# isabella232/kyverno

Measured on AMD Instinct MI355X. Metric: resource×rule validate evals/sec (node), higher is better.
Workload: dtype u8; 1 GPU; C2: synthetic Pods x 100 validate.pattern rules (image globs, ?*, quantities, |-lists); rules=100, pairs_per_gpu=100000000, output=full, parallelism=resource-shard x1, engine=specialized

## Files before the change

kyverno_amd/csrc/kvdevfn.h:

```cpp
#pragma once

#define KV_SENT 0xFFFFFFFFu


#ifdef KV_JIT_PRELUDE
#define KV_FN __device__ __forceinline__
#define KV_GLOB_FN __device__ __forceinline__
#else
#define KV_FN __device__
#define KV_GLOB_FN __device__ __noinline__
#endif

__device__ __forceinline__ uint32_t uni(uint32_t v) { return __builtin_amdgcn_readfirstlane(v); }

#ifndef KV_SCONST
#define KV_SCONST __attribute__((address_space(4)))
#endif
template <class T>
__device__ __forceinline__ T sld(const T* p) {
  static_assert(sizeof(T) % 4 == 0, "sld: whole words");
  const KV_SCONST uint32_t* q = (const KV_SCONST uint32_t*)p;
  uint32_t w[sizeof(T) / 4];
#pragma unroll
  for (uint32_t i = 0; i < sizeof(T) / 4; i++) w[i] = q[i];
// ... 601 lines not shown
  uint32_t kind, flags, pn, key, res, i0, i1, i2, i3;
};

__device__ __forceinline__ uint2 err8_pack(uint32_t kind, uint32_t flags, uint32_t pn, uint32_t key, uint32_t i0,
                                           uint32_t i1, uint32_t i2, uint32_t i3, uint32_t r) {
  const uint32_t fits = (i0 < 1024u) & (i1 < 256u) & (i2 < 256u) & (i3 == 0u) & (key == ABSENT) & (pn < (1u << 25));
  uint2 w;
  w.x = kind | (flags << 4) | ((fits ^ 1u) << 6) | (pn << 7);
  w.y = (i0 & 1023u) | ((i1 & 255u) << 10) | ((i2 & 255u) << 18) | ((r & 63u) << 26);
  return w;
}

__device__ __forceinline__ void store_err(const DevOut& O, uint32_t ri, uint32_t n_res, uint32_t r, uint32_t kind,
                                          uint32_t flags, uint32_t pn, uint32_t key, uint32_t res, uint32_t i0,
                                          uint32_t i1, uint32_t i2, uint32_t i3) {
#if defined(KV_JIT_PRELUDE) && !defined(KVEMU)
  if (KV_OFULL(O) & 4) return;
#else
  if (KV_OFULL(O) & 4) {
    uint4* x = (uint4*)(O.err + (size_t)ri * n_res) + 2u * r;
    x[0] = make_uint4(kind | (flags << 16), pn, key, res);
    x[1] = make_uint4(i0, i1, i2, i3);
    return;
  }
#endif
  ((uint2*)(O.err8 + (size_t)ri * n_res))[r] = err8_pack(kind, flags, pn, key, i0, i1, i2, i3, r);
}

__device__ __forceinline__ uint32_t kv_count_bytes(uint32_t w, uint32_t b4) {
  const uint32_t t = w ^ b4;
  return (uint32_t)__popc(~(((t & 0x7F7F7F7Fu) + 0x7F7F7F7Fu) | t | 0x7F7F7F7Fu));
}

__device__ __forceinline__ uint32_t kv_ptab_col(const DevPS& P, uint32_t type, uint32_t a) {
  if (type - 1u < 4u) return a;
  return P.n_vals - KV_PTAB_PSEUDO + (type == NT_NULL ? 0u : type == NT_MAP ? 1u : 2u);
}

__device__ __forceinline__ uint32_t kv_leaf_word(const DevPS& P, const Node* __restrict__ N, const Node& n, uint32_t w) {
  const uint32_t t = node_type(n.kt);
#ifdef KV_DIAG_XPTAB
  if (t != NT_ARR) return (n.a * 0x9E3779B9u) ^ (w * 0x85EBCA6Bu);
#endif
  if (t != NT_ARR) return kv_gld(P.ptab, (size_t)w * P.n_vals + kv_ptab_col(P, t, n.a));
  uint32_t x = 0xFFFFFFFFu;
  for (uint32_t k = 0; k < n.b; k++) {
    const Node e = N[ni(n.a + k)];
    x &= kv_gld(P.ptab, (size_t)w * P.n_vals + kv_ptab_col(P, node_type(e.kt), e.a));
  }
  return x;
}

__device__ __forceinline__ uint32_t kv_leaf_word_n(const DevPS& P, const Node* __restrict__ N, const Node& n, uint32_t w) {
  const uint32_t t = node_type(n.kt);
  if (t != NT_ARR) return kv_leaf_word(P, N, n, w);
  const uint32_t ai = ni(n.a);
  const uint32_t first = kv_gld(&N[ai].a, 0), count = kv_gld(&N[ai].b, 0);
  uint32_t x = 0xFFFFFFFFu;
  for (uint32_t k = 0; k < count; k++) {
    const Node e = N[ni(first + k)];
    x &= kv_gld(P.ptab, (size_t)w * P.n_vals + kv_ptab_col(P, node_type(e.kt), e.a));
  }
  return x;
}

__device__ __forceinline__ void kv_rec_put(const DevOut& O, uint32_t ri, uint32_t n_res, uint32_t r, uint32_t slot,
                                           const EState& e, uint32_t z) {
#ifdef KV_DIAG_NORECST
  asm volatile("" ::"v"(slot));
  return;
#endif
  ((uint2*)(O.err8 + (size_t)ri * n_res))[(r & ~63u) + (slot & 63u)] =
      err8_pack(e.kind + z, e.flags, e.pn + z, e.key + z, e.i0, e.i1, e.i2, e.i3, r);
}

__device__ __forceinline__ void kv_final(const DevOut& O, uint32_t ri, uint32_t n_res, uint32_t r, bool valid,
                                         uint32_t st, const EState& e, uint8_t* s_row, uint32_t row) {
#ifdef KV_DIAG_NOREC
  if (false) {
#else
  if (valid && (KV_OFULL(O) & 2) && (st == ST_FAIL || st == ST_ERROR || st == ST_SKIP)) {
#endif
    uint32_t z = 0u;
#ifndef KVEMU
    asm volatile("" : "+v"(r), "+v"(z));
    asm volatile("" : "+s"(ri));
#endif
#if defined(KV_JIT_PRELUDE) && !defined(KVEMU)
    if (!(KV_OFULL(O) & 4)) {
      uint8_t* s_c = s_row - KV_ROW0 - row * KV_RSTRIDE + __builtin_amdgcn_readfirstlane(threadIdx.x >> 6) * KV_KROWS;
      const uint32_t sh = 8u * (row & 3u);
      kv_rec_put(O, ri, n_res, r, atomicAdd((uint32_t*)(s_c + (row & ~3u)), 1u << sh) >> sh, e, z);
    }
#else
    store_err(O, ri, n_res, r, e.kind + z, e.flags, e.pn + z, e.key + z, e.res + z, e.i0, e.i1, e.i2, e.i3);
#endif
// ... 257 lines not shown
```

kyverno_amd/csrc/kvjit.hpp:

```cpp
#pragma once
#include <cstdint>
#include <map>
#include <string>
#include <vector>

#include "kvinternal.hpp"
#include "kvdevtypes.h"

namespace kvh {

struct JitChunk {
  std::vector<uint32_t> rules;
  std::string name;
};

struct JitKernelPlan {
  uint32_t first, count;
  int waves;
  std::vector<uint32_t> blocks;
};

struct JitImage {
  std::vector<JitKernelPlan> plan;
  std::string source;
  std::string common;
  std::vector<std::string> kernel_name, kernel_src;
  std::vector<std::vector<char>> codes;
  std::vector<JitChunk> chunks;
  std::vector<uint32_t> memo_preds;
  uint32_t memo_words = 0;
  uint32_t ptab_row = 1;
  uint32_t mtup_words = 0;
  std::vector<uint32_t> fac_word, fac_bit, fac_flist, fac_rule;
  uint32_t fac_slots = 0;
  std::vector<uint8_t> rec_compact;
  std::vector<uint32_t> gs_desc, gs_mem;
  uint32_t gs_members = 0;
  std::vector<kv::ColDesc> cols;
  std::vector<uint32_t> fam_arr, fam_ncols;
  std::vector<uint32_t> fam_nw, fam_nb, fam_nn;
  std::map<std::string, uint32_t> col_use;
  bool probe = false;
  double gen_ms = 0, compile_ms = 0;
  struct Variant {
    uint32_t full = 0;
    std::vector<std::vector<char>> codes;
  };
  std::vector<Variant> variants;
};

uint32_t jit_chunk_rules();
constexpr uint32_t kJitStamps = 16;
// ... 19 lines not shown
```

kyverno_amd/csrc/kvjitbuild.cpp:

```cpp
#include <hip/hiprtc.h>

#include <dlfcn.h>
#include <sched.h>
#include <spawn.h>
#include <sys/stat.h>
#include <sys/wait.h>

#include <cerrno>
#include <unistd.h>

#include <algorithm>
#include <atomic>
#include <chrono>
#include <cstdio>
#include <cstdlib>
#include <cstring>
#include <set>
#include <sstream>
#include <stdexcept>
#include <thread>

#include "kvjit.hpp"

extern char** environ;
// ... 236 lines not shown
bool reg_verdict(const JitImage& img, size_t ci, int waves, RegVerdict* out) {
  uint32_t priv = 0, vgprs = 0;
  if (ci >= img.codes.size() || !co_kernel_info(img.codes[ci], img.kernel_name[ci], &priv, &vgprs)) return false;
  *out = reg_verdict_of(priv, vgprs, waves, img.kernel_src[ci].find("kv_dleaf_impl") != std::string::npos);
  return true;
}

std::string variant_common(const JitImage& img, uint32_t full) {
  return "#define KVJ_FULL " + std::to_string(full) + "u\n" + img.common;
}

}

RegVerdict reg_verdict_of(uint32_t priv, uint32_t vgprs, int waves, bool calls) {
  RegVerdict v{priv, vgprs, calls, false, false};
  v.fits = waves == 0 || vgprs <= 512u / (uint32_t)waves;
  v.scratch_ok = priv == 0 || (calls && waves == 0);
  return v;
}

bool jit_plan_spills(JitImage* img, const std::vector<RegVerdict>& verdicts) {
  std::vector<JitKernelPlan> next;
  bool changed = false;
  for (size_t k = 0; k < img->plan.size(); k++) {
    const JitKernelPlan& kp = img->plan[k];
    const RegVerdict& v = verdicts.at(k);
    if (v.ships()) {
      next.push_back(kp);
      continue;
    }
    changed = true;
    JitKernelPlan np = kp;
    const size_t big = (size_t)(std::max_element(np.blocks.begin(), np.blocks.end()) - np.blocks.begin());
    if (v.calls && v.fits) {
      np.waves = 0;
    } else if (kp.waves > 6 && np.blocks.size() > 1) {
      np.waves = kp.waves - 1;
    } else if (!np.blocks.empty() && np.blocks[big] > 1) {
      const uint32_t c = np.blocks[big], h = c / 2;
      np.blocks[big] = h;
      np.blocks.insert(np.blocks.begin() + big + 1, c - h);
    } else if (kp.waves > 1) {
      np.waves = kp.waves - 1;
    } else if (kp.waves == 1) {
      np.waves = 0;
    } else if (kp.count > 1) {
      const uint32_t h = kp.count / 2;
      next.push_back({kp.first, h, 0, std::vector<uint32_t>(h, 1u)});
      next.push_back({kp.first + h, kp.count - h, 0, std::vector<uint32_t>(kp.count - h, 1u)});
      continue;
    } else {
      throw std::runtime_error("kvjit: kernel " + img->chunks[k].name + " needs " + std::to_string(v.priv) +
                               " B of scratch per lane even without a launch bound");
    }
    next.push_back(np);
  }
  if (changed) img->plan = next;
  return changed;
}

namespace {

bool jit_plan_spills(JitImage* img) {
  std::vector<RegVerdict> verdicts(img->plan.size());
  for (size_t k = 0; k < img->plan.size(); k++)
    if (!reg_verdict(*img, program_of(*img, img->chunks[k].name), img->plan[k].waves, &verdicts[k]))
      throw std::runtime_error("kvjit: no kernel descriptor for " + img->chunks[k].name);
// ... 66 lines not shown
        else nb.push_back(c);
      }
      img->plan[k].blocks = nb;
    }
  }
}

std::string jit_plan_key(const JitImage& img) {
  uint64_t h = common_hash(img.common);
  for (size_t i = 0; i < img.kernel_src.size(); i++) h = fnv1a64(img.kernel_src[i], fnv1a64(img.kernel_name[i], h));
  char key[40];
  snprintf(key, sizeof key, "%016llx", (unsigned long long)h);
  return key;
}

}

uint64_t code_bytes(const JitImage& img) {
  uint64_t n = 0;
  for (auto& c : img.codes) n += c.size();
  return n;
}

bool jit_load_plan(const std::string& key, JitImage* img) {
  const std::string dir = cache_dir();
  std::vector<char> text;
  if (dir.empty() || !read_file(dir + "/plan-" + key + ".txt", &text)) return false;
  std::vector<JitKernelPlan> plan;
  std::istringstream in(std::string(text.begin(), text.end()));
  for (std::string line; std::getline(in, line);) {
    if (line.rfind("kernel ", 0) != 0) continue;
    std::istringstream ls(line.substr(7));
    JitKernelPlan kp{0, 0, 0, {}};
    ls >> kp.first >> kp.count >> kp.waves;
    uint32_t sum = 0;
    for (uint32_t b; ls >> b; sum += b) kp.blocks.push_back(b);
    if (sum != kp.count || kp.blocks.empty()) return false;
    plan.push_back(kp);
  }
  if (plan.empty()) return false;
  img->plan = plan;
  return true;
}

void jit_save_plan(const std::string& key, const JitImage& img) {
  const std::string dir = cache_dir();
  if (dir.empty()) return;
  std::string t;
  for (const JitKernelPlan& kp : img.plan) {
    t += "kernel " + std::to_string(kp.first) + " " + std::to_string(kp.count) + " " + std::to_string(kp.waves);
    for (uint32_t b : kp.blocks) t += " " + std::to_string(b);
    t += "\n";
  }
  const uint64_t hc = common_hash(img.common);
  for (size_t i = 0; i < img.kernel_src.size(); i++) t += "co " + cache_file(img, i, hc) + "\n";
  for (const JitImage::Variant& v : img.variants) {
    const uint64_t hv = common_hash(variant_common(img, v.full));
    for (size_t i = 0; i < img.kernel_src.size(); i++)
      if (i < v.codes.size() && !v.codes[i].empty()) t += "co " + cache_file(img, i, hv) + "\n";
  }
  write_file_atomic(dir, dir + "/plan-" + key + ".txt", t);
}

void jit_build(const PolicySet& ps, JitImage* img) {
  const uint32_t chunk = jit_chunk_rules();
  const char* dump = getenv("KVGPU_JIT_DUMP");
  jit_generate(ps, chunk, img);
  if (dump) write_file(dump, img->source);
  if (!getenv("KVGPU_JIT_SKIP_COMPILE")) {
    const std::string pkey = jit_plan_key(*img);
    if (!jit_load_plan(pkey, img)) jit_refine_blocks(ps, chunk, img);
    jit_generate(ps, chunk, img);
    bool settled = false;
    for (int round = 0; round < 64 && !settled; round++) {
      jit_compile(img);
      settled = !jit_plan_spills(img);
      if (!settled) jit_generate(ps, chunk, img);
    }
    if (!settled)
      throw std::runtime_error("kvjit: the register plan did not settle (kernels still spill after 64 re-plans)");
    jit_compile_variants(img);
    jit_save_plan(pkey, *img);
    if (dump) write_file(dump, img->source);
  }
  if (const char* co = getenv("KVGPU_JIT_DUMP_CO")) {
    for (size_t i = 0; i < img->codes.size(); i++) write_file(std::string(co) + "." + img->kernel_name[i] + ".co", img->codes[i]);
    for (const JitImage::Variant& v : img->variants)
      for (size_t i = 0; i < v.codes.size(); i++)
        if (!v.codes[i].empty())
          write_file(std::string(co) + "." + img->kernel_name[i] + ".m" + std::to_string(v.full) + ".co", v.codes[i]);
  }
}

}
```

kyverno_amd/csrc/kvjitgen.cpp:

```cpp
#include <algorithm>
#include <chrono>
#include <cstdio>
#include <cstdlib>
#include <cstring>
#include <map>
#include <set>
#include <sstream>
#include <stdexcept>
#include <unordered_map>

#include "kvjit.hpp"
#include "kvdevtypes.h"

namespace kvh {

using namespace kv;

namespace {

const char* kPrelude =
#include "kvjit_prelude.inc"
    ;

std::string hex32(uint32_t v) {
// ... 46 lines not shown
  struct Form {
    std::string text;
    std::vector<uint32_t> preds, pns;
    std::vector<uint32_t> leafpcs;
  };

  const PolicySet& ps;
  const GenOpts opt;

  std::vector<uint32_t> mpreds;
  std::map<uint32_t, uint32_t> pslot;
  std::map<uint32_t, uint32_t> pmask;
  std::vector<Fam> fams;
  std::map<std::string, uint32_t> fam_of;
  std::map<std::string, uint32_t> use_seed;
  std::vector<uint32_t> gs_desc, gs_mem;
  uint32_t gs_members = 0;
  std::vector<uint32_t> mt_bits;
  std::vector<uint8_t> rec_slot;
  uint32_t gtab_n = 0;
  std::map<uint32_t, Form> forms;
  std::map<uint32_t, uint32_t> bslot;
  std::map<uint32_t, std::set<uint32_t>> glob_bytes;
  std::vector<std::pair<std::string, std::string>> helpers;
  std::set<uint32_t> globs_done, atoms_done, preds_done, blks_done;
  std::set<std::pair<char, uint32_t>> qglobs_done, qatoms_done, qpreds_done;
  bool dleaf_done = false;
  std::vector<std::pair<std::string, std::string>> kernels;

  struct Kern {
    uint32_t mt_kbase = 0;
    uint32_t gs0 = 0, gsn = 0;
    std::string decls;
  };

  explicit Gen(const PolicySet& p) : ps(p), rec_slot(p.rules.size(), 0) {
    fams.emplace_back();
    col_of(0, "R");
  }

  struct Helper : std::ostringstream {
    Gen& g;
    const std::string name;
    Helper(Gen& gg, std::string n) : g(gg), name(std::move(n)) {}
    ~Helper() { g.helpers.push_back({name, str()}); }
  };
  static std::string num(const char* prefix, uint32_t i) { return prefix + std::to_string(i); }

  enum ColUse : uint32_t { CU_WIDE = 1u, CU_B = 2u, CU_LEAF = 4u };
  void col_mark(int fam, uint32_t j, uint32_t use) {
    if (fam >= 0 && j != kNoCol) fams.at((size_t)fam).use.at(j) |= use;
  }
  static std::string col_macro(const char* what, uint32_t f, uint32_t j) {
    return std::string("KVC_") + what + "_" + std::to_string(f) + "_" + std::to_string(j);
  }
  static constexpr uint32_t kNoCol = 0xFFFFFFFFu;
  static bool expr_steps(const std::string& ex, std::vector<uint32_t>* out) {
    out->clear();
    size_t at = ex.find('/');
    while (at != std::string::npos) {
      const size_t nx = ex.find('/', at + 1);
      const std::string tok = ex.substr(at + 1, nx == std::string::npos ? std::string::npos : nx - at - 1);
      if (tok.size() < 2 || (tok[0] != 's' && tok[0] != 'k')) return false;
      const unsigned long v = strtoul(tok.c_str() + 1, nullptr, 10);
      if (v >= KV_COL_SCAN) return false;
      out->push_back((uint32_t)v | (tok[0] == 'k' ? KV_COL_SCAN : 0u));
// ... 3 lines not shown
  }
  uint32_t col_of(uint32_t f, const std::string& rel) {
    Fam& F = fams.at(f);
    auto it = F.idx.find(rel);
    if (it != F.idx.end()) return it->second;
    std::vector<uint32_t> st;
    if (!expr_steps(rel, &st)) return kNoCol;
    const uint32_t j = (uint32_t)F.steps.size();
    F.idx.emplace(rel, j);
    F.steps.push_back(st);
    F.use.push_back(0u);
    return j;
  }
  uint32_t family(const std::string& arr) {
    auto it = fam_of.find(arr);
    if (it != fam_of.end()) return it->second;
    if (col_of(0, arr) == kNoCol) return kNoCol;
    const uint32_t f = (uint32_t)fams.size();
    fams.emplace_back();
    fams.back().arr = arr;
    col_of(f, "");
    fam_of.emplace(arr, f);
    return f;
  }
  void col_plan(JitImage* out, std::string* defs) const {
    out->cols.clear();
    out->fam_arr.clear();
    out->fam_ncols.clear();
    out->fam_nw.clear();
    out->fam_nb.clear();
    out->fam_nn.clear();
    out->col_use.clear();
    std::ostringstream d;
    for (uint32_t f = 0; f < fams.size(); f++) {
      const Fam& F = fams[f];
      out->fam_arr.push_back(f ? fams[0].idx.at(F.arr) : 0u);
      out->fam_ncols.push_back((uint32_t)F.steps.size());
      std::vector<uint32_t> use(F.steps.size(), 0u);
      for (const auto& kv : F.idx) {
        const std::string key = F.arr + "|" + kv.first;
        uint32_t u = F.use[kv.second];
        auto it = use_seed.find(key);
        if (it != use_seed.end()) u |= it->second;
        if (f == 0 && fam_of.count(kv.first)) u |= CU_WIDE | CU_B;
        use[kv.second] = u;
        out->col_use[key] = u;
      }
      uint32_t nw = 0, nb = 0, nn = 0;
      const size_t c0 = out->cols.size();
      for (uint32_t j = 0; j < F.steps.size(); j++) {
        ColDesc c{};
        c.fam = f;
        c.j = j;
        c.nsteps = (uint32_t)F.steps[j].size();
        for (uint32_t s = 0; s < c.nsteps; s++) c.steps[s] = F.steps[j][s];
        if (opt.narrow && !(use[j] & CU_WIDE)) {
          c.fmt = KV_COLF_NARROW;
          c.pos = nn++;
        } else {
          c.pos = nw++;
          c.fmt = KV_COLF_WIDE;
          if (use[j] & (CU_B | CU_LEAF)) {
            c.fmt = KV_COLF_WIDEB;
            c.bpos = nb++;
          }
        }
        out->cols.push_back(c);
      }
      out->fam_nw.push_back(nw);
      out->fam_nb.push_back(nb);
      out->fam_nn.push_back(nn);
      d << "#define KVC_W" << f << " " << (3u * nw + nb + nn) * KV_LANES << "u\n";
      for (uint32_t j = 0; j < F.steps.size(); j++) {
        const ColDesc& c = out->cols[c0 + j];
        d << "#define " << col_macro("LD", f, j) << "(b) ";
        if (c.fmt == KV_COLF_NARROW) {
          d << "kv_ldn(PC, (b) + " << u32((3u * nw + nb + c.pos) * KV_LANES) << " + ln_)\n"
            << "#define " << col_macro("IX", f, j) << "(n) (node_type((n).kt) == NT_MAP ? KV_NARROW_IDX : 0u)\n"
            << "#define " << col_macro("LW", f, j) << "(n, w) kv_leaf_word_n(P, N, n, w)\n";
        } else {
          if (c.fmt == KV_COLF_WIDEB)
            d << "kv_ldwb(PC, (b) + " << u32(c.pos * 3u * KV_LANES) << " + 3u * ln_, (b) + "
              << u32((3u * nw + c.bpos) * KV_LANES) << " + ln_)\n";
          else
            d << "kv_ldw(PC, (b) + " << u32(c.pos * 3u * KV_LANES) << " + 3u * ln_)\n";
          d << "#define " << col_macro("IX", f, j) << "(n) (node_type((n).kt) == NT_MAP ? (n).c : 0u)\n"
            << "#define " << col_macro("LW", f, j) << "(n, w) kv_leaf_word(P, N, n, w)\n";
        }
      }
    }
    for (uint32_t f = 1; f < fams.size(); f++) out->cols.at(out->fam_arr[f]).arr_fam = f;
    *defs = d.str();
  }

  template <class Fn>
  void each_atom(uint32_t pi, Fn fn) const {
    const Pred& pr = ps.preds[pi];
    if (pr.kind != PK_STRING) return;
    for (uint32_t a = pr.first; a < pr.first + pr.count; a++)
      for (uint32_t c = ps.alts[a].first; c < ps.alts[a].first + ps.alts[a].count; c++) {
        fn(ps.conjs[c].a0);
        if (ps.conjs[c].kind != CJ_ATOM) fn(ps.conjs[c].a1);
      }
  }

  std::string seg_expr(const GSeg& sg, const std::string& k, bool aligned0) {
    const uint32_t nw = (sg.len + 3) / 4;
    std::ostringstream e;
    e << "([&]() -> bool { ";
    if (aligned0) {
      e << "uint32_t x = 0u; ";
      for (uint32_t i = 0; i < nw; i++) {
        const GWord& g = ps.gwords[sg.wfirst + i];
        if (g.mask == 0) continue;
        e << "x |= (base[" << i << "] ^ " << hex32(g.w) << ") & " << hex32(g.mask) << "; ";
      }
      e << "return x == 0u; })()";
      return e.str();
    }
    e << "const uint32_t k_ = " << k << ", a_ = k_ >> 2, sh_ = k_ & 3u; uint32_t lo_ = base[a_], hi_, x = 0u; ";
// ... 542 lines not shown
    for (uint32_t f = rr.m_first; f < rr.m_first + rr.m_count; f++) blk_fn(f);
    for (uint32_t f = rr.x_first; f < rr.x_first + rr.x_count; f++) blk_fn(f);
    auto call = [&](uint32_t f) { return "g_blk_" + std::to_string(f) + "(P, B, R, rkind, rflags)"; };
    auto combine = [&](uint32_t mode, uint32_t first, uint32_t count) {
      std::ostringstream e;
      if (mode == 0 || count == 0) {
        e << call(first);
      } else {
        e << "(";
        for (uint32_t f = first; f < first + count; f++) e << (f > first ? (mode == 1 ? " || " : " && ") : "") << call(f);
        e << ")";
      }
      return e.str();
    };
    Helper o(*this, num("g_match_", ri));
    o << "__device__ __forceinline__ bool " << o.name
      << "(const DevPS& P, const DevBatch& B, const Res* __restrict__ R, uint32_t rkind, uint32_t rflags) {\n"
      << "  if (!" << combine(rr.m_mode, rr.m_first, rr.m_count) << ") return false;\n"
      << "  return !" << combine(rr.x_mode, rr.x_first, rr.x_count) << ";\n}\n";
  }

  static uint32_t prog_end(const PolicySet& ps, uint32_t pc) {
    while ((ps.prog[pc].op & 0xFF) != OP_DONE) pc++;
    return pc;
  }

  static constexpr uint32_t FIN = 0x7F000000u, ACT = 0x80000000u;

  struct HVar {
    std::string idx, node;
    int fam = -1;
    uint32_t j = kNoCol;
  };
  struct HoistTable {
    std::string prefix;
    std::map<std::string, HVar> vars;
    std::vector<std::string> code;
    std::set<std::string> words;
    size_t flushed = 0;
    uint32_t n = 0;
    int fam = -1;
    std::string troot, cell0;
    std::string flush() {
      std::string s;
      for (; flushed < code.size(); flushed++) s += code[flushed];
      return s;
    }
  };

  struct RGen {
    uint32_t ri = 0, b = 0, e = 0, maxd = 1;
    std::vector<std::pair<uint32_t, uint32_t>> loops;
    std::vector<std::string> expr;
    std::vector<HVar> hv;
    std::vector<std::vector<std::pair<int, uint32_t>>> csrc;
    std::set<uint32_t> resume;
    std::set<uint32_t> carry_ok, carry_err;
    std::vector<char> lean, post_alt;
    std::vector<uint32_t> post_flags, skip_to;
    uint32_t q = 0;
    bool uses_anchor = false, uses_keyglob = false;
    bool grp = false;
    uint32_t gn = 1, grow = 0, gsri = 0, gspn = 0;
    std::vector<uint32_t> gri, gdpn;
    std::map<uint32_t, uint32_t> gslot;
    std::string gtab;
    bool gsite = false;
    uint32_t gl = 0, gpre = 0;
    uint32_t max_level = 0;
    std::string s;
  };

  HVar hoist(HoistTable& T, const std::string& pexpr, const HVar& p, uint32_t a, uint32_t aux) {
    const bool scan = (aux & AUX_SCAN) != 0;
    const std::string ex = pexpr + (scan ? "/k" : "/s") + std::to_string(a);
    auto it = T.vars.find(ex);
    if (it != T.vars.end()) return it->second;
    HVar h{T.prefix + "h" + std::to_string(T.n), T.prefix + "hn" + std::to_string(T.n)};
    T.n++;
    std::ostringstream c;
    const uint32_t j = T.fam >= 0 ? col_of((uint32_t)T.fam, T.fam == 0 ? ex : ex.substr(T.troot.size())) : kNoCol;
    if (j != kNoCol) {
      h.fam = T.fam;
      h.j = j;
      c << "  const Node " << h.node << " = " << col_macro("LD", (uint32_t)T.fam, j) << "(" << T.cell0 << ");\n"
        << "  const uint32_t " << h.idx << " = " << h.node << ".kt == 0u ? ABSENT : "
        << col_macro("IX", (uint32_t)T.fam, j) << "(" << h.node << ");\n";
      T.code.push_back(c.str());
      T.vars.emplace(ex, h);
      return h;
    }
    col_mark(p.fam, p.j, CU_WIDE | CU_B);
    c << "  uint32_t " << h.idx << " = ABSENT; Node " << h.node << "{0u, 0u, 0u, 0u};\n";
    if (scan) {
      c << "  if (node_type(" << p.node << ".kt) == NT_MAP) for (uint32_t q_ = 0u; q_ < " << p.node << ".b; q_++) { "
        << "const uint32_t c_ = ni(" << p.node << ".a + q_); const Node t_ = N[c_]; if (node_key(t_.kt) == " << u32(a)
        << ") { " << h.idx << " = c_; " << h.node << " = t_; break; } }\n";
    } else {
      c << "  { const bool ok_ = node_type(" << p.node << ".kt) == NT_MAP && " << u32(a) << " < " << p.node << ".b; "
        << "const uint32_t c_ = ok_ ? ni(" << p.node << ".a + " << u32(a) << ") : 0u; const Node t_ = N[c_]; "
        << "const bool hit_ = ok_ && node_type(t_.kt) != NT_ABSENT; const uint32_t m_ = hit_ ? 0x07060504u : 0x0c0c0c0cu; "
        << h.idx << " = hit_ ? c_ : ABSENT; " << h.node << " = Node{__builtin_amdgcn_perm(t_.kt, 0u, m_), "
        << "__builtin_amdgcn_perm(t_.a, 0u, m_), __builtin_amdgcn_perm(t_.b, 0u, m_), __builtin_amdgcn_perm(t_.c, 0u, m_)}; }\n";
    }
    T.code.push_back(c.str());
    T.vars.emplace(ex, h);
    return h;
  }

  struct Region {
    int kind = 0;
    uint32_t rb = 0, re = 0;
    uint32_t jre = 0;
    std::string se;
    std::set<uint32_t>*jumps = nullptr, *err_jumps = nullptr;
    std::string li0;
    HoistTable* T = nullptr;
    std::string troot;
  };

  struct GInfo {
    std::vector<uint32_t> members, pns0, leafpcs;
    std::vector<uint32_t> dpn;
    std::vector<std::vector<uint32_t>> preds;
  };

  struct Block {
    Kern& kern;
    const uint32_t hbase;
    std::vector<uint32_t> rules;
    std::vector<GInfo> ginfo;
    std::map<uint32_t, size_t> gof;
    std::vector<RGen> gs;
    HoistTable global;
    size_t K = 0;
    Block(Kern& k, uint32_t hb) : kern(k), hbase(hb) {
      global.prefix = "g";
      global.fam = 0;
// ... 152 lines not shown
        case OP_KEYGLOB:
          if (G) throw std::runtime_error("kvjit: KEYGLOB in a rule group");
          set_unknown(d + 1);
          IDX(d);
          w << "  { uint32_t nd_; if (!keyglob_op(P, B, N, " << cd << ", " << u32(in.op) << ", " << u32(in.a) << ", "
            << u32(in.c) << ", &nd_, &kn" << s << ")) " << jump(in.b) << " " << cn << " = nd_; }\n";
          break;
        case OP_SCOPE_END:
          if (G) break;
          if (in.c == 0) w << "  if (" << kindof << ") " << ek << " |= " << u32(aux << 4) << ";\n";
          else w << "  if (" << kindof << ") { " << ek << " |= " << u32(aux << 4) << "; " << jump(in.c, true) << " }\n";
          break;
        case OP_POS_END:
          if (G) throw std::runtime_error("kvjit: POS_END in a rule group");
          w << "  if (" << kindof << ") { if (" << ek << " & " << u32(EF_COND << 4) << ") " << ek << " = 0u; else "
            << jump(in.c, true) << " }\n";
          break;
        case OP_NEG:
          w << "  if (" << lookup(d, in.a, aux, false) << " != ABSENT) " << raise(E_NEG, in.b, in.c) << "\n";
          break;
        case OP_STAR:
          w << "  if (" << absent_or(d + 1, "== NT_NULL") << ") " << raise(E_STAR, in.b, in.c) << "\n";
          break;
        case OP_LEAF: {
          const uint32_t slot = G ? g.gslot.at(pc) : slot_for(in.a);
          const uint32_t word = slot / 32;
          HoistTable* T = known(d) ? table_for(d) : nullptr;
          std::string wx;
          if (T) {
            const HVar& hvd = g.hv[d];
            const std::string hn = hvd.node;
            wx = hn + "_w" + std::to_string(word);
            col_mark(hvd.fam, hvd.j, CU_LEAF);
            if (T->words.insert(wx).second)
              T->code.push_back("  const uint32_t " + wx + " = " +
                                (hvd.fam >= 0 ? col_macro("LW", (uint32_t)hvd.fam, hvd.j) + "(" + hn + ", "
                                              : "kv_leaf_word(P, N, " + hn + ", ") +
                                u32(word) + ");\n");
          } else {
            IDX(d);
            wx = "kv_leaf_word(P, N, (" + cd + " != ABSENT ? N[" + cd + "] : Node{0u, 0u, 0u, 0u}), " + u32(word) + ")";
          }
          if (G) {
            const uint32_t mask = g.gn >= 32 ? 0xFFFFFFFFu : (1u << g.gn) - 1u;
            w << "  { const uint32_t f_ = " << al << " & ~((" << wx << " >> " << u32(slot % 32) << ") & " << hex32(mask)
              << ");\n    if (f_) { " << gfin("f_", E_VALUE, in.b, in.c) << " " << al << " &= ~f_; if (!" << al << ") "
              << gdone() << " } }\n";
          } else {
            w << "  if (!(((" << wx << " >> " << u32(slot % 32) << ") & 1u) != 0u)) " << raise(E_VALUE, in.b, in.c) << "\n";
          }
          break;
        }
        case OP_VLEAF:
          if (G) throw std::runtime_error("kvjit: VLEAF in a rule group");
          if (known(d)) w << "  { const Node vn_ = " << NODE(d, CU_WIDE | CU_B) << ";\n";
          else {
            IDX(d);
            w << "  { Node vn_{0u, 0u, 0u, 0u}; if (" << cd << " != ABSENT) vn_ = N[" << cd << "];\n";
          }
          dleaf_fn();
          w << "    if (!g_dleaf_0(B, N, B.dleaf[(size_t)" << u32(in.a) << " * n_res + r], vn_)) "
            << raise(E_VALUE, in.b, in.c) << " }\n";
          break;
        case OP_RAISE:
          w << "  " << raise(in.b, in.a, in.c) << "\n";
          break;
        case OP_EXISTCHK:
          w << "  if (" << absent_or(d, "!= NT_ARR") << ") " << raise(E_EXIST_RESTYPE, in.a, in.c) << "\n";
          break;
        case OP_LENCHK:
          w << "  if (" << NODE(d, CU_WIDE | CU_B) << ".b < " << u32(in.a) << ") " << raise(E_LEN, in.b, in.c) << "\n";
// ... 557 lines not shown
    }
    Loop L;
    L.k = k;
    L.tag = tag;
    L.troot = "E" + tag;
    L.T.prefix = "l" + tag + "_";
    L.fam = key[0] == 'R' && fams[0].idx.count(key) ? family(key) : kNoCol;
    if (L.fam != kNoCol) {
      L.T.fam = (int)L.fam;
      L.T.troot = L.troot;
      L.T.cell0 = "ec" + tag;
    }
    std::ostringstream bodies;
    for (RGen* gp : grp) loop_body(B, *gp, L, bodies);
    std::vector<uint32_t> gmask(B.mask_words(), 0);
    for (const RGen* gp : grp)
      if (gp->lean[k]) gmask[gp->q / 32] |= 1u << (gp->q % 32);
    body << "  { // fused loop " << tag << " over " << key << " (" << grp.size() << " rules)\n"
         << "    uint32_t fn" << tag << " = 0u, ff" << tag << " = 0u, fe" << tag << " = 0u;\n    if (((0u";
    for (const RGen* gp : grp)
      if (!gp->lean[k]) body << " | rs" << gp->s;
    body << ") & ACT_)";
    for (uint32_t w = 0; w < gmask.size(); w++)
      if (gmask[w]) body << " | (am" << k << "_" << w << " & " << u32(gmask[w]) << ")";
    body << ") { const Node an_ = " << arr_node << "; ff" << tag << " = an_.a; fn" << tag << " = an_.b; fe" << tag
         << " = an_.c; }\n";
    body << "    for (uint32_t fli" << tag << " = 0u; fli" << tag << " < fn" << tag << "; fli" << tag << "++) {\n"
         << "      const uint32_t el" << tag << " = ni(ff" << tag << " + fli" << tag << ");\n";
    if (L.fam != kNoCol)
      body << "      const uint32_t ec" << tag << " = fe" << tag << " + fli" << tag << " * KVC_W" << L.fam
           << ";\n      const Node eln" << tag << " = " << col_macro("LD", L.fam, 0) << "(ec" << tag << ");\n";
    else
      body << "      const Node eln" << tag << " = N[el" << tag << "];\n";
    body << L.T.flush() << bodies.str() << "    }\n";
    for (const RGen* gp : grp)
      if (!gp->lean[k]) body << "    rs" << gp->s << " &= ~ACT_;\n";
    body << "  }\n";
  }

  void emit_fused_loops(Block& B, size_t k, std::ostream& body) {
    std::map<std::string, std::vector<RGen*>> groups;
    std::vector<std::string> order;
    for (RGen& g : B.gs) {
      if (k >= g.loops.size()) continue;
      const uint32_t d = (ps.prog[g.loops[k].first].op >> 8) & 0xFF;
      const std::string key = g.expr[d].empty() ? "U" + std::to_string(g.ri) : g.expr[d];
      if (!groups.count(key)) order.push_back(key);
      groups[key].push_back(&g);
    }
    uint32_t li = 0;
    for (const std::string& key : order) emit_fused_loop(B, k, key, groups[key], std::to_string(k) + "_" + std::to_string(li++), body);
  }

  void emit_rule_state(const Block& B, std::ostream& k) const {
    for (uint32_t ri : B.rules)
      if (!B.gof.count(ri)) k << "  uint32_t rs_" << ri << " = FIN_ | ST_NOMATCH;\n";
    for (const RGen& g : B.gs) {
      const std::string& s = g.s;
      if (g.grp) k << "  uint32_t rs" << s << " = FIN_ | ST_STORED_, al" << s << " = 0u;\n";
      k << "  uint32_t ek" << s << " = 0u";
      for (uint32_t lv = 0; lv <= g.max_level && lv < 4; lv++) k << ", ei" << lv << s << " = 0u";
      if (g.uses_keyglob) k << ", kn" << s << " = ABSENT, ekn" << s << " = ABSENT";
      k << ";\n";
      if (g.uses_anchor) k << "  uint64_t areg" << s << " = 0ull, apres" << s << " = 0ull;\n";
      k << "  uint32_t c0" << s << " = root";
      for (uint32_t d = 1; d < g.maxd; d++) k << ", c" << d << s << " = ABSENT";
      k << ";\n";
      k << "  uint32_t";
      for (uint32_t l = 0; l <= g.max_level && l < 4; l++)
        k << (l ? "," : "") << " li" << l << s << " = 0u, lf" << l << s << " = 0u, ll" << l << s << " = 0u";
      k << ";\n";
    }
  }

  static void check_resumes(const Block& B) {
    for (const RGen& g : B.gs)
      for (uint32_t t : g.resume) {
        bool ok = false;
        for (size_t k = 0; k <= g.loops.size() && !ok; k++) ok = t >= segment(g, k).first && t < segment(g, k).second;
        if (!ok) throw std::runtime_error("kvjit: resume target " + std::to_string(t) + " of rule " +
                                         std::to_string(g.ri) + " is not in a segment");
      }
  }

  std::string fused_block(Kern& kern, const std::vector<uint32_t>& rules_in, uint32_t hbase, std::vector<uint32_t>* order) {
    Block B(kern, hbase);
    form_groups(rules_in, &B);
    *order = B.rules;
    prepare_rules(&B);
    std::ostringstream body;
    for (size_t k = 0; k <= B.K; k++) {
      std::ostringstream seg;
      for (RGen& g : B.gs)
        if (k <= g.loops.size()) emit_segment(B, g, k, seg);
      if (k < B.K) {
        body << "  uint32_t";
        for (uint32_t w = 0; w < B.mask_words(); w++)
          body << (w ? "," : "") << " am" << k << "_" << w << " = 0u, sk" << k << "_" << w << " = 0u";
        body << ";\n";
      }
      body << B.global.flush() << seg.str();
      if (k < B.K) emit_fused_loops(B, k, body);
    }
    check_resumes(B);
    std::ostringstream k;
    emit_rule_state(B, k);
    for (uint32_t q = 0; q < B.rules.size(); q++)
      if (no_program(ps.rules[B.rules[q]])) k << match_code(B, q) << store(B, q);
    k << body.str();
    return k.str();
  }

  static uint32_t kernel_lds(uint32_t nr) { return KV_ROW0 + nr * KV_RSTRIDE; }
  static int lds_waves(uint32_t nr) {
    const uint32_t g = 1280u, b = (kernel_lds(nr) + g - 1u) / g * g;
    return (int)std::max<uint32_t>(1u, (160u * 1024u) / std::max(b, g) * KV_RWAVES / 4u);
  }
  std::vector<uint32_t> group_kernel(const std::string& name, const std::vector<std::vector<uint32_t>>& chs, int waves) {
    std::vector<std::string> blocks;
    std::vector<std::pair<uint32_t, uint32_t>> rows;
    std::vector<uint32_t> rules;
    uint32_t nr_all = 0;
    for (const auto& c : chs) nr_all += (uint32_t)c.size();
    if (nr_all > KV_KROWS) throw std::runtime_error("kvjit: at most KV_KROWS rules per kernel (KVGPU_JIT_CHUNK)");
    Kern kern;
    kern.mt_kbase = (uint32_t)(mt_bits.size() / 32u);
    kern.gs0 = (uint32_t)(gs_desc.size() / 4u);
    for (const auto& c : chs) {
      std::vector<uint32_t> ord;
      rows.push_back({(uint32_t)rules.size(), (uint32_t)c.size()});
      blocks.push_back(fused_block(kern, c, (uint32_t)rules.size(), &ord));
      rules.insert(rules.end(), ord.begin(), ord.end());
    }
    mt_bits.insert(mt_bits.end(), rules.begin(), rules.end());
    while (mt_bits.size() % 32u) mt_bits.push_back(0xFFFFFFFFu);
    const uint32_t nr = (uint32_t)rules.size();
    if (kern.gsn > 64u) throw std::runtime_error("kvjit: more than 64 site-record groups in one kernel");
    std::ostringstream o;
    o << kern.decls;
    if (opt.stamps) o << "__device__ unsigned long long* kvj_stamps;\n";
    o << "__device__ const uint32_t " << name << "_rules[" << nr << "] = {";
    for (uint32_t q = 0; q < nr; q++) o << (q ? ", " : "") << u32(rules[q]);
    o << "};\n";
    const std::string lb = waves > 0 ? "KV_RWG, " + std::to_string(waves) : "KV_RWG";
    o << "extern \"C\" __global__ __launch_bounds__(" << lb << ") void " << name
      << "(const DevPS* __restrict__ Pp, const DevBatch* __restrict__ Bp, const Node* __restrict__ N, "
         "const Val* __restrict__ V, const uint8_t* __restrict__ S, DevOut O, uint32_t r0) {\n"
      << "  constexpr uint32_t FIN_ = " << u32(FIN) << ", ACT_ = " << u32(ACT) << ", ST_STORED_ = 0x7Eu;\n"
      << "  __shared__ unsigned long long s_stq[" << kernel_lds(nr) / 8 + (KV_RWAVES * kern.gsn + 1u) / 2u
      << "];\n  uint32_t* s_stw = (uint32_t*)s_stq;\n"
      << "  const DevPS& P = *Pp;\n  const DevBatch& B = *Bp;\n  const uint8_t* __restrict__ pstr = P.pstr;\n";
    o << "  const uint32_t nb_ = gridDim.x, x_ = blockIdx.x & 7u, per_ = nb_ >> 3, rem_ = nb_ & 7u;\n"
      << "  const uint32_t bx_ = x_ * per_ + (x_ < rem_ ? x_ : rem_) + (blockIdx.x >> 3);\n";
    o << "  const uint32_t r = r0 + bx_ * KV_RWG + threadIdx.x;\n"
      << "  const uint32_t n_res = B.n_res;\n"
      << "  const bool valid = r < n_res;\n"
      << "  const Res* __restrict__ R = B.res + (valid ? r : 0u);\n"
      << "  uint32_t root = ABSENT, rkind = KEY_NONE, rflags = 0u, rtup = 0u;\n"
      << "  if (valid) { root = ni(kv_gld(&R->root, 0)); rkind = kv_gld(&R->kind, 0); rflags = kv_gld(&R->flags, 0); rtup = kv_gld(&R->tup, 0); }\n"
      << "  Node rootn{0u, 0u, 0u, 0u};\n";
// ... 201 lines not shown
      const KindSpec& k = ps.kinds[i];
      if (k.form == 3) return "*";
      ks.push_back(std::to_string(k.kind));
    }
  }
  std::sort(ks.begin(), ks.end());
  ks.erase(std::unique(ks.begin(), ks.end()), ks.end());
  std::string key;
  for (auto& k : ks) key += k + ",";
  return key;
}

std::vector<uint32_t> rule_order(const PolicySet& ps) {
  std::vector<std::pair<std::string, uint32_t>> order;
  for (uint32_t ri = 0; ri < ps.rules.size(); ri++)
    order.push_back({!no_program(ps.rules[ri]) ? "0" + rule_kind_key(ps, ri) + "#" + rule_signature(ps, ri) : "1", ri});
  std::stable_sort(order.begin(), order.end());
  std::vector<uint32_t> sorted;
  for (auto& o : order) sorted.push_back(o.second);
  return sorted;
}

std::vector<JitKernelPlan> first_plan(Gen& g, const std::vector<uint32_t>& sorted, uint32_t chunk_rules) {
  const uint32_t n = (uint32_t)sorted.size();
  if (chunk_rules == 0 || chunk_rules > KV_KROWS) chunk_rules = KV_KROWS;
  uint32_t parts = (n + chunk_rules - 1) / chunk_rules;
  while (parts < n && Gen::lds_waves((n + parts - 1) / parts) < Gen::lds_waves(n / parts)) parts++;
  std::vector<JitKernelPlan> plan;
  for (uint32_t k = 0; k < parts; k++) {
    const uint32_t a = (uint32_t)((uint64_t)n * k / parts), e = (uint32_t)((uint64_t)n * (k + 1) / parts);
    std::vector<uint32_t> bl = g.initial_blocks(sorted, a, e);
    const int lds_waves = Gen::lds_waves(e - a);
    const int rule_waves = (int)std::max<uint32_t>(1u, (160u * 1024u) / std::max<uint32_t>(1u, (e - a) * 256u));
    plan.push_back({a, e - a, g.opt.has_waves ? g.opt.waves : std::min({8, lds_waves, rule_waves}), bl});
  }
  return plan;
}

void assemble_programs(const Gen& g, const std::string& prelude, const std::string& cdefs, JitImage* out) {
  const std::vector<std::pair<std::string, std::string>>& defs = g.helpers;
  std::unordered_map<std::string, size_t> def_index;
  for (size_t i = 0; i < defs.size(); i++) def_index[defs[i].first] = i;
  auto refs = [&](const std::string& text, std::vector<size_t>* out_ids) {
    static const char* prefixes[] = {"g_glob_", "g_atom_", "g_pred_", "g_blk_", "g_match_",
                                     "g_dleaf_", "q_glob_", "q_atom_", "q_pred_", "r_glob_", "r_atom_", "r_pred_"};
    for (const char* pf : prefixes) {
      const size_t pl = strlen(pf);
      for (size_t q = text.find(pf); q != std::string::npos; q = text.find(pf, q + pl)) {
        size_t e = q + pl;
        while (e < text.size() && isdigit((unsigned char)text[e])) e++;
        auto it = def_index.find(text.substr(q, e - q));
        if (it != def_index.end()) out_ids->push_back(it->second);
      }
    }
  };
  out->common = prelude;
  out->kernel_name.clear();
  out->kernel_src.clear();
  out->source = prelude + cdefs;
  for (const auto& d : defs) out->source += d.second;
  for (auto& k : g.kernels) {
    std::vector<char> used(defs.size(), 0);
    std::vector<size_t> stack;
    refs(k.second, &stack);
    while (!stack.empty()) {
      const size_t d = stack.back();
      stack.pop_back();
// ... 14 lines not shown

uint32_t jit_chunk_rules() {
  const char* ch = getenv("KVGPU_JIT_CHUNK");
  return ch && atoi(ch) > 0 ? std::min<uint32_t>((uint32_t)atoi(ch), KV_KROWS) : KV_KROWS;
}

void jit_generate(const PolicySet& ps, uint32_t chunk_rules, JitImage* out) {
  auto t0 = std::chrono::steady_clock::now();
  Gen g(ps);
  g.use_seed = out->col_use;
  const std::string prelude =
      g.opt.diag + kPrelude + std::string("\nusing namespace kv;\n\n") +
      "__device__ __noinline__ bool kv_dleaf_impl(const DevBatch& B, const Node* __restrict__ N, uint32_t dp, Node vn);\n\n";
  for (uint32_t ri = 0; ri < ps.rules.size(); ri++)
    if (!no_program(ps.rules[ri])) g.leaf_classes(ri);
  for (uint32_t ri = 0; ri < ps.rules.size(); ri++) g.match_fn(ri);
  out->chunks.clear();
  const uint32_t n = (uint32_t)ps.rules.size();
  const std::vector<uint32_t> sorted = rule_order(ps);
  if (out->plan.empty() && n) out->plan = first_plan(g, sorted, chunk_rules);
  for (const JitKernelPlan& kp : out->plan) {
    JitChunk kc;
    kc.name = "kvj_r" + std::to_string(kp.first) + "_" + std::to_string(kp.count) +
              (kp.blocks.size() > 1 ? "_b" + std::to_string(kp.blocks.size()) : "") + (kp.waves ? "" : "u");
    for (uint32_t q = kp.first; q < kp.first + kp.count; q++) kc.rules.push_back(sorted.at(q));
    std::vector<std::vector<uint32_t>> bl;
    uint32_t at = 0;
    for (uint32_t c : kp.blocks) {
      if (at + c > kp.count) break;
      bl.emplace_back(kc.rules.begin() + at, kc.rules.begin() + at + c);
      at += c;
    }
    if (at != kp.count) throw std::runtime_error("kvjit: kernel plan blocks do not cover its rules");
    kc.rules = g.group_kernel(kc.name, bl, kp.waves);
    out->chunks.push_back(kc);
  }
  out->mtup_words = (uint32_t)(g.mt_bits.size() / 32u);
  if (out->mtup_words && !out->probe) g.build_fac(out);
  out->rec_compact.assign(n, 1);
  for (uint32_t ri = 0; ri < n; ri++) out->rec_compact[ri] = g.rec_slot[ri] ? 0 : 1;
  out->gs_desc = g.gs_desc;
  out->gs_mem = g.gs_mem;
  out->gs_members = g.gs_members;
  std::string cdefs;
  g.col_plan(out, &cdefs);

  out->memo_preds.clear();
  out->memo_words = 0;
  if (!g.mpreds.empty() && !out->probe) {
    g.ptab_kernel();
    out->memo_preds = g.mpreds;
    out->memo_words = (uint32_t)((g.mpreds.size() + 31) / 32);
    out->ptab_row = g.ptab_row_out();
  }
  assemble_programs(g, prelude, cdefs, out);
  out->gen_ms = std::chrono::duration<double, std::milli>(std::chrono::steady_clock::now() - t0).count();
}

}
```

Baseline: 297.6 billion evals/s.

## Batch hoisted leaf-word gathers and defer array fixups behind a wave ballot

The JIT code generator now emits the hoisted ptab leaf-word loads as plain single gathers grouped together after the cell loads. The rarely needed array-node AND-loop is moved into one block guarded by a wave-wide ballot. This lets the independent global loads issue back to back instead of interleaving with branches and loops per word. The grouped form is tried after the register plan settles and is dropped per kernel if it would spill, at the cost of an extra generate and compile pass and a new field in the plan-cache format.

```diff
diff --git a/kyverno_amd/csrc/kvdevfn.h b/kyverno_amd/csrc/kvdevfn.h
--- a/kyverno_amd/csrc/kvdevfn.h
+++ b/kyverno_amd/csrc/kvdevfn.h
@@ -657,9 +657,22 @@
   return (uint32_t)__popc(~(((t & 0x7F7F7F7Fu) + 0x7F7F7F7Fu) | t | 0x7F7F7F7Fu));
 }
 
+__device__ __forceinline__ uint32_t kv_ptab_col(uint32_t n_vals, uint32_t type, uint32_t a) {
+  if (type - 1u < 4u) return a;
+  return n_vals - KV_PTAB_PSEUDO + (type == NT_NULL ? 0u : type == NT_MAP ? 1u : 2u);
+}
 __device__ __forceinline__ uint32_t kv_ptab_col(const DevPS& P, uint32_t type, uint32_t a) {
-  if (type - 1u < 4u) return a;
-  return P.n_vals - KV_PTAB_PSEUDO + (type == NT_NULL ? 0u : type == NT_MAP ? 1u : 2u);
+  return kv_ptab_col(P.n_vals, type, a);
+}
+
+__device__ __forceinline__ uint32_t kv_arr_word(const uint32_t* __restrict__ ptab, uint32_t n_vals,
+                                                const Node* __restrict__ N, uint32_t first, uint32_t count, uint32_t w) {
+  uint32_t x = 0xFFFFFFFFu;
+  for (uint32_t k = 0; k < count; k++) {
+    const Node e = N[ni(first + k)];
+    x &= kv_gld(ptab, (size_t)w * n_vals + kv_ptab_col(n_vals, node_type(e.kt), e.a));
+  }
+  return x;
 }
 
 __device__ __forceinline__ uint32_t kv_leaf_word(const DevPS& P, const Node* __restrict__ N, const Node& n, uint32_t w) {
@@ -668,25 +681,28 @@
   if (t != NT_ARR) return (n.a * 0x9E3779B9u) ^ (w * 0x85EBCA6Bu);
 #endif
   if (t != NT_ARR) return kv_gld(P.ptab, (size_t)w * P.n_vals + kv_ptab_col(P, t, n.a));
-  uint32_t x = 0xFFFFFFFFu;
-  for (uint32_t k = 0; k < n.b; k++) {
-    const Node e = N[ni(n.a + k)];
-    x &= kv_gld(P.ptab, (size_t)w * P.n_vals + kv_ptab_col(P, node_type(e.kt), e.a));
-  }
-  return x;
+  return kv_arr_word(P.ptab, P.n_vals, N, n.a, n.b, w);
+}
+
+__device__ __forceinline__ uint32_t kv_leaf_gather(const DevPS& P, const Node& n, uint32_t w) {
+#ifdef KV_DIAG_XPTAB
+  if (node_type(n.kt) != NT_ARR) return (n.a * 0x9E3779B9u) ^ (w * 0x85EBCA6Bu);
+#endif
+  return kv_gld(P.ptab, (size_t)w * P.n_vals + kv_ptab_col(P, node_type(n.kt), n.a));
+}
+__device__ __forceinline__ uint32_t kv_leaf_fix(const uint32_t* __restrict__ ptab, uint32_t n_vals, const Node* __restrict__ N,
+                                             uint32_t a, uint32_t b, bool narrow, uint32_t w) {
+  if (narrow) {
+    const uint32_t ai = ni(a);
+    a = kv_gld(&N[ai].a, 0);
+    b = kv_gld(&N[ai].b, 0);
+  }
+  return kv_arr_word(ptab, n_vals, N, a, b, w);
 }
 
 __device__ __forceinline__ uint32_t kv_leaf_word_n(const DevPS& P, const Node* __restrict__ N, const Node& n, uint32_t w) {
-  const uint32_t t = node_type(n.kt);
-  if (t != NT_ARR) return kv_leaf_word(P, N, n, w);
-  const uint32_t ai = ni(n.a);
-  const uint32_t first = kv_gld(&N[ai].a, 0), count = kv_gld(&N[ai].b, 0);
-  uint32_t x = 0xFFFFFFFFu;
-  for (uint32_t k = 0; k < count; k++) {
-    const Node e = N[ni(first + k)];
-    x &= kv_gld(P.ptab, (size_t)w * P.n_vals + kv_ptab_col(P, node_type(e.kt), e.a));
-  }
-  return x;
+  if (node_type(n.kt) != NT_ARR) return kv_leaf_word(P, N, n, w);
+  return kv_leaf_fix(P.ptab, P.n_vals, N, n.a, 0u, true, w);
 }
 
 __device__ __forceinline__ void kv_rec_put(const DevOut& O, uint32_t ri, uint32_t n_res, uint32_t r, uint32_t slot,
diff --git a/kyverno_amd/csrc/kvjit.hpp b/kyverno_amd/csrc/kvjit.hpp
--- a/kyverno_amd/csrc/kvjit.hpp
+++ b/kyverno_amd/csrc/kvjit.hpp
@@ -18,6 +18,7 @@
   uint32_t first, count;
   int waves;
   std::vector<uint32_t> blocks;
+  bool grouped = false;
 };
 
 struct JitImage {
diff --git a/kyverno_amd/csrc/kvjitbuild.cpp b/kyverno_amd/csrc/kvjitbuild.cpp
--- a/kyverno_amd/csrc/kvjitbuild.cpp
+++ b/kyverno_amd/csrc/kvjitbuild.cpp
@@ -292,7 +292,9 @@
     changed = true;
     JitKernelPlan np = kp;
     const size_t big = (size_t)(std::max_element(np.blocks.begin(), np.blocks.end()) - np.blocks.begin());
-    if (v.calls && v.fits) {
+    if (kp.grouped) {
+      np.grouped = false;
+    } else if (v.calls && v.fits) {
       np.waves = 0;
     } else if (kp.waves > 6 && np.blocks.size() > 1) {
       np.waves = kp.waves - 1;
@@ -425,7 +427,7 @@
     if (line.rfind("kernel ", 0) != 0) continue;
     std::istringstream ls(line.substr(7));
     JitKernelPlan kp{0, 0, 0, {}};
-    ls >> kp.first >> kp.count >> kp.waves;
+    ls >> kp.first >> kp.count >> kp.waves >> kp.grouped;
     uint32_t sum = 0;
     for (uint32_t b; ls >> b; sum += b) kp.blocks.push_back(b);
     if (sum != kp.count || kp.blocks.empty()) return false;
@@ -441,7 +443,8 @@
   if (dir.empty()) return;
   std::string t;
   for (const JitKernelPlan& kp : img.plan) {
-    t += "kernel " + std::to_string(kp.first) + " " + std::to_string(kp.count) + " " + std::to_string(kp.waves);
+    t += "kernel " + std::to_string(kp.first) + " " + std::to_string(kp.count) + " " + std::to_string(kp.waves) + " " +
+         (kp.grouped ? "1" : "0");
     for (uint32_t b : kp.blocks) t += " " + std::to_string(b);
     t += "\n";
   }
@@ -453,6 +456,25 @@
       if (i < v.codes.size() && !v.codes[i].empty()) t += "co " + cache_file(img, i, hv) + "\n";
   }
   write_file_atomic(dir, dir + "/plan-" + key + ".txt", t);
+}
+
+static void jit_group_regions(const PolicySet& ps, uint32_t chunk, JitImage* img) {
+  for (JitKernelPlan& kp : img->plan) kp.grouped = true;
+  jit_generate(ps, chunk, img);
+  jit_compile(img);
+  bool back = false;
+  for (size_t k = 0; k < img->plan.size(); k++) {
+    RegVerdict v;
+    if (!reg_verdict(*img, program_of(*img, img->chunks[k].name), img->plan[k].waves, &v))
+      throw std::runtime_error("kvjit: no kernel descriptor for " + img->chunks[k].name);
+    if (!v.ships()) {
+      img->plan[k].grouped = false;
+      back = true;
+    }
+  }
+  if (!back) return;
+  jit_generate(ps, chunk, img);
+  jit_compile(img);
 }
 
 void jit_build(const PolicySet& ps, JitImage* img) {
@@ -462,7 +484,11 @@
   if (dump) write_file(dump, img->source);
   if (!getenv("KVGPU_JIT_SKIP_COMPILE")) {
     const std::string pkey = jit_plan_key(*img);
-    if (!jit_load_plan(pkey, img)) jit_refine_blocks(ps, chunk, img);
+    const bool stored = jit_load_plan(pkey, img);
+    if (!stored) {
+      for (JitKernelPlan& kp : img->plan) kp.grouped = false;
+      jit_refine_blocks(ps, chunk, img);
+    }
     jit_generate(ps, chunk, img);
     bool settled = false;
     for (int round = 0; round < 64 && !settled; round++) {
@@ -472,6 +498,7 @@
     }
     if (!settled)
       throw std::runtime_error("kvjit: the register plan did not settle (kernels still spill after 64 re-plans)");
+    if (!stored) jit_group_regions(ps, chunk, img);
     jit_compile_variants(img);
     jit_save_plan(pkey, *img);
     if (dump) write_file(dump, img->source);
diff --git a/kyverno_amd/csrc/kvjitgen.cpp b/kyverno_amd/csrc/kvjitgen.cpp
--- a/kyverno_amd/csrc/kvjitgen.cpp
+++ b/kyverno_amd/csrc/kvjitgen.cpp
@@ -102,6 +102,7 @@
     uint32_t mt_kbase = 0;
     uint32_t gs0 = 0, gsn = 0;
     std::string decls;
+    bool grouped = false;
   };
 
   explicit Gen(const PolicySet& p) : ps(p), rec_slot(p.rules.size(), 0) {
@@ -171,6 +172,9 @@
     out->fam_nn.clear();
     out->col_use.clear();
     std::ostringstream d;
+    d << "#define KVC_LO_ROW(n, w) kv_leaf_word(P, N, n, w)\n"
+      << "#define KVC_LW_ROW(n, w) kv_leaf_gather(P, n, w)\n"
+      << "#define KVC_LA_ROW(n, w) kv_leaf_fix(P.ptab, P.n_vals, N, (n).a, (n).b, false, w)\n";
     for (uint32_t f = 0; f < fams.size(); f++) {
       const Fam& F = fams[f];
       out->fam_arr.push_back(f ? fams[0].idx.at(F.arr) : 0u);
@@ -216,7 +220,9 @@
         if (c.fmt == KV_COLF_NARROW) {
           d << "kv_ldn(PC, (b) + " << u32((3u * nw + nb + c.pos) * KV_LANES) << " + ln_)\n"
             << "#define " << col_macro("IX", f, j) << "(n) (node_type((n).kt) == NT_MAP ? KV_NARROW_IDX : 0u)\n"
-            << "#define " << col_macro("LW", f, j) << "(n, w) kv_leaf_word_n(P, N, n, w)\n";
+            << "#define " << col_macro("LO", f, j) << "(n, w) kv_leaf_word_n(P, N, n, w)\n"
+            << "#define " << col_macro("LW", f, j) << "(n, w) kv_leaf_gather(P, n, w)\n"
+            << "#define " << col_macro("LA", f, j) << "(n, w) kv_leaf_fix(P.ptab, P.n_vals, N, (n).a, 0u, true, w)\n";
         } else {
           if (c.fmt == KV_COLF_WIDEB)
             d << "kv_ldwb(PC, (b) + " << u32(c.pos * 3u * KV_LANES) << " + 3u * ln_, (b) + "
@@ -224,7 +230,9 @@
           else
             d << "kv_ldw(PC, (b) + " << u32(c.pos * 3u * KV_LANES) << " + 3u * ln_)\n";
           d << "#define " << col_macro("IX", f, j) << "(n) (node_type((n).kt) == NT_MAP ? (n).c : 0u)\n"
-            << "#define " << col_macro("LW", f, j) << "(n, w) kv_leaf_word(P, N, n, w)\n";
+            << "#define " << col_macro("LO", f, j) << "(n, w) kv_leaf_word(P, N, n, w)\n"
+            << "#define " << col_macro("LW", f, j) << "(n, w) kv_leaf_gather(P, n, w)\n"
+            << "#define " << col_macro("LA", f, j) << "(n, w) kv_leaf_fix(P.ptab, P.n_vals, N, (n).a, (n).b, false, w)\n";
         }
       }
     }
@@ -833,19 +841,57 @@
     int fam = -1;
     uint32_t j = kNoCol;
   };
+  struct HWord {
+    std::string var;
+    HVar hv;
+    uint32_t word = 0;
+  };
   struct HoistTable {
     std::string prefix;
     std::map<std::string, HVar> vars;
-    std::vector<std::string> code;
-    std::set<std::string> words;
-    size_t flushed = 0;
+    std::vector<std::string> cells;
+    std::vector<HWord> words;
+    std::vector<char> order;
+    std::set<std::string> have;
+    size_t cflushed = 0, wflushed = 0, oflushed = 0;
+    void add_cell(const std::string& c) { cells.push_back(c); order.push_back('c'); }
+    void add_word(const HWord& w) { words.push_back(w); order.push_back('w'); }
     uint32_t n = 0;
     int fam = -1;
     std::string troot, cell0;
-    std::string flush() {
+    std::string flush(bool grouped) {
       std::string s;
-      for (; flushed < code.size(); flushed++) s += code[flushed];
-      return s;
+      if (!grouped) {
+        for (; oflushed < order.size(); oflushed++) {
+          if (order[oflushed] == 'c') {
+            s += cells[cflushed++];
+            continue;
+          }
+          const HWord& x = words[wflushed++];
+          s += "  const uint32_t " + x.var + " = " +
+               (x.hv.fam >= 0 ? col_macro("LO", (uint32_t)x.hv.fam, x.hv.j) : std::string("KVC_LO_ROW")) + "(" + x.hv.node +
+               ", " + std::to_string(x.word) + "u);\n";
+        }
+        return s;
+      }
+      oflushed = order.size();
+      for (; cflushed < cells.size(); cflushed++) s += cells[cflushed];
+      if (wflushed == words.size()) return s;
+      std::vector<std::string> nodes;
+      std::string fix;
+      for (size_t i = wflushed; i < words.size(); i++) {
+        const HWord& x = words[i];
+        const bool col = x.hv.fam >= 0;
+        const std::string args = "(" + x.hv.node + ", " + std::to_string(x.word) + "u);\n";
+        s += "  uint32_t " + x.var + " = " + (col ? col_macro("LW", (uint32_t)x.hv.fam, x.hv.j) : std::string("KVC_LW_ROW")) + args;
+        if (std::find(nodes.begin(), nodes.end(), x.hv.node) == nodes.end()) nodes.push_back(x.hv.node);
+        fix += "    if (node_type(" + x.hv.node + ".kt) == NT_ARR) " + x.var + " = " +
+               (col ? col_macro("LA", (uint32_t)x.hv.fam, x.hv.j) : std::string("KVC_LA_ROW")) + args;
+      }
+      wflushed = words.size();
+      s += "  if (__ballot(";
+      for (size_t i = 0; i < nodes.size(); i++) s += (i ? " || " : "") + ("node_type(" + nodes[i] + ".kt) == NT_ARR");
+      return s + ") != 0ull) {  // some leaf cell is an array (rare)\n" + fix + "  }\n";
     }
   };
 
@@ -887,7 +933,7 @@
       c << "  const Node " << h.node << " = " << col_macro("LD", (uint32_t)T.fam, j) << "(" << T.cell0 << ");\n"
         << "  const uint32_t " << h.idx << " = " << h.node << ".kt == 0u ? ABSENT : "
         << col_macro("IX", (uint32_t)T.fam, j) << "(" << h.node << ");\n";
-      T.code.push_back(c.str());
+      T.add_cell(c.str());
       T.vars.emplace(ex, h);
       return h;
     }
@@ -904,7 +950,7 @@
         << h.idx << " = hit_ ? c_ : ABSENT; " << h.node << " = Node{__builtin_amdgcn_perm(t_.kt, 0u, m_), "
         << "__builtin_amdgcn_perm(t_.a, 0u, m_), __builtin_amdgcn_perm(t_.b, 0u, m_), __builtin_amdgcn_perm(t_.c, 0u, m_)}; }\n";
     }
-    T.code.push_back(c.str());
+    T.add_cell(c.str());
     T.vars.emplace(ex, h);
     return h;
   }
@@ -1123,11 +1169,7 @@
             const std::string hn = hvd.node;
             wx = hn + "_w" + std::to_string(word);
             col_mark(hvd.fam, hvd.j, CU_LEAF);
-            if (T->words.insert(wx).second)
-              T->code.push_back("  const uint32_t " + wx + " = " +
-                                (hvd.fam >= 0 ? col_macro("LW", (uint32_t)hvd.fam, hvd.j) + "(" + hn + ", "
-                                              : "kv_leaf_word(P, N, " + hn + ", ") +
-                                u32(word) + ");\n");
+            if (T->have.insert(wx).second) T->add_word(HWord{wx, hvd, word});
           } else {
             IDX(d);
             wx = "kv_leaf_word(P, N, (" + cd + " != ABSENT ? N[" + cd + "] : Node{0u, 0u, 0u, 0u}), " + u32(word) + ")";
@@ -1751,7 +1793,7 @@
            << ";\n      const Node eln" << tag << " = " << col_macro("LD", L.fam, 0) << "(ec" << tag << ");\n";
     else
       body << "      const Node eln" << tag << " = N[el" << tag << "];\n";
-    body << L.T.flush() << bodies.str() << "    }\n";
+    body << L.T.flush(B.kern.grouped) << bodies.str() << "    }\n";
     for (const RGen* gp : grp)
       if (!gp->lean[k]) body << "    rs" << gp->s << " &= ~ACT_;\n";
     body << "  }\n";
@@ -1818,7 +1860,7 @@
           body << (w ? "," : "") << " am" << k << "_" << w << " = 0u, sk" << k << "_" << w << " = 0u";
         body << ";\n";
       }
-      body << B.global.flush() << seg.str();
+      body << B.global.flush(B.kern.grouped) << seg.str();
       if (k < B.K) emit_fused_loops(B, k, body);
     }
     check_resumes(B);
@@ -1835,7 +1877,8 @@
     const uint32_t g = 1280u, b = (kernel_lds(nr) + g - 1u) / g * g;
     return (int)std::max<uint32_t>(1u, (160u * 1024u) / std::max(b, g) * KV_RWAVES / 4u);
   }
-  std::vector<uint32_t> group_kernel(const std::string& name, const std::vector<std::vector<uint32_t>>& chs, int waves) {
+  std::vector<uint32_t> group_kernel(const std::string& name, const std::vector<std::vector<uint32_t>>& chs, int waves,
+                                     bool grouped) {
     std::vector<std::string> blocks;
     std::vector<std::pair<uint32_t, uint32_t>> rows;
     std::vector<uint32_t> rules;
@@ -1845,6 +1888,7 @@
     Kern kern;
     kern.mt_kbase = (uint32_t)(mt_bits.size() / 32u);
     kern.gs0 = (uint32_t)(gs_desc.size() / 4u);
+    kern.grouped = grouped;
     for (const auto& c : chs) {
       std::vector<uint32_t> ord;
       rows.push_back({(uint32_t)rules.size(), (uint32_t)c.size()});
@@ -2112,7 +2156,7 @@
     std::vector<uint32_t> bl = g.initial_blocks(sorted, a, e);
     const int lds_waves = Gen::lds_waves(e - a);
     const int rule_waves = (int)std::max<uint32_t>(1u, (160u * 1024u) / std::max<uint32_t>(1u, (e - a) * 256u));
-    plan.push_back({a, e - a, g.opt.has_waves ? g.opt.waves : std::min({8, lds_waves, rule_waves}), bl});
+    plan.push_back({a, e - a, g.opt.has_waves ? g.opt.waves : std::min({8, lds_waves, rule_waves}), bl, true});
   }
   return plan;
 }
@@ -2193,7 +2237,7 @@
       at += c;
     }
     if (at != kp.count) throw std::runtime_error("kvjit: kernel plan blocks do not cover its rules");
-    kc.rules = g.group_kernel(kc.name, bl, kp.waves);
+    kc.rules = g.group_kernel(kc.name, bl, kp.waves, kp.grouped);
     out->chunks.push_back(kc);
   }
   out->mtup_words = (uint32_t)(g.mt_bits.size() / 32u);
```

Measured after the change: 328.0 billion evals/s (median of 6 runs). 10.2% higher.
